# haoxiangsnr/Wave-U-Net-for-Speech-Enhancement

Hardware: AMD Instinct MI355X
Metric: 16384-sample frames/sec fwd+bwd, 12-level Wave-U-Net (higher is better)
Workload: dtype f32 (levels >= 16 samples: 3 x f16 MFMA on hi/lo fp16 halves, fp32 accumulate; the rest f32 MFMA); 1 GPU; unet_basic 12-level, 16384-sample frames, batch=64 per GPU, fp32, training-mode forward + smooth_l1 + backward + fused HIP Adam step (BASELINE.json configs[2]; configs[3] when n_gpus>1); global_batch=64, frame=16384, parallelism=dp1

## Files before the change

include/wunet_hip.h:

```cpp
#ifndef WUNET_HIP_H
#define WUNET_HIP_H

#include <stddef.h>

#ifdef __cplusplus
extern "C" {
#endif

typedef struct wunet_ctx wunet_ctx;

#define WUNET_OK 0
#define WUNET_E_ARG (-1)
#define WUNET_E_RUNTIME (-2)

#define WUNET_LOSS_MSE 0
#define WUNET_LOSS_L1 1
#define WUNET_LOSS_SMOOTH_L1 2

const char* wunet_last_error(void);

int wunet_create(int n_layers, int channels_interval, int batch, int length, wunet_ctx** out);
void wunet_destroy(wunet_ctx* ctx);

int wunet_set_h3(wunet_ctx* ctx, int enable);
// ... 13 lines not shown
                   float* const* grads, void* stream);
int wunet_backward_range(wunet_ctx* ctx, const float* noisy, const float* const* params,
                         const float* enhanced, const float* grad_enhanced, void* workspace,
                         float* const* grads, int layer_begin, int layer_end, void* stream);
int wunet_backward_range_async(wunet_ctx* ctx, const float* noisy, const float* const* params,
                               const float* enhanced, const float* grad_enhanced, void* workspace,
                               float* const* grads, int layer_begin, int layer_end, void* stream);
int wunet_backward_join(wunet_ctx* ctx, void* stream);
int wunet_backward_input(wunet_ctx* ctx, const float* noisy, const float* const* params, void* workspace,
                         float* grad_noisy, void* stream);

size_t wunet_loss_scratch_bytes(void);
int wunet_loss_forward(int kind, const float* clean, const float* enhanced, size_t n,
                       float* loss_out, void* scratch, void* stream);
int wunet_loss_backward(int kind, const float* clean, const float* enhanced, const float* grad_loss,
                        size_t n, float* grad_enhanced, void* stream);

int wunet_adam_step(int n_tensors, float* const* params, const float* const* grads, float* const* exp_avg,
                    float* const* exp_avg_sq, const size_t* numels, double lr, double beta1, double beta2, double eps,
                    long long step, double grad_scale, long long* step_dev, float* hyper_dev, void* stream);

int wunet_layer_info(const wunet_ctx* ctx, int layer, size_t* z_offset_floats, int* channels, int* length);
int wunet_num_conv_layers(const wunet_ctx* ctx);

int wunet_profile_enable(int on);
long long wunet_profile_collect(char* buf, size_t cap);
int wunet_debug_stamps(unsigned long long* out, int n);

#define WUNET_COMM_ID_BYTES 128
typedef struct wunet_comm wunet_comm;
int wunet_comm_unique_id(unsigned char* id );
int wunet_comm_create(const unsigned char* id, int world, int rank, wunet_comm** out);
int wunet_comm_allreduce_sum(wunet_comm* comm, float* buf, size_t count, void* stream);
int wunet_comm_world(const wunet_comm* comm);
void wunet_comm_destroy(wunet_comm* comm);

int wunet_crop_windows(const float* mixture_flat, const float* clean_flat, const long long* starts, long long total,
                       int batch, int length, float* mixture, float* clean, void* stream);

void wunet_debug_set_conv_trace(void* dev_buffer);

int wunet_op_conv1d(const float* x, const float* w, const float* bias, float* z,
                    int B, int Cin, int Cout, int L, int K, void* stream);
int wunet_op_conv1d_dgrad(const float* gz, const float* w, float* dx,
                          int B, int Cin, int Cout, int L, int K, void* stream);
int wunet_op_conv1d_wgrad(const float* gz, const float* x, float* dw,
// ... 14 lines not shown
```

wave-u-net-for-speech-enhancement_amd/_lib.py:

```python
import ctypes
import os

_HERE = os.path.dirname(os.path.abspath(__file__))
LIB_PATH = os.environ.get("WUNET_LIB_PATH") or os.path.join(_HERE, "csrc", "libwunet_hip.so")

EXPORTS = [
    "wunet_last_error", "wunet_create", "wunet_destroy", "wunet_workspace_bytes", "wunet_forward",
    "wunet_backward", "wunet_backward_range", "wunet_loss_scratch_bytes", "wunet_loss_forward",
    "wunet_loss_backward", "wunet_layer_info", "wunet_num_conv_layers", "wunet_op_conv1d",
    "wunet_op_conv1d_dgrad", "wunet_op_conv1d_wgrad", "wunet_profile_enable", "wunet_profile_collect",
    "wunet_adam_step", "wunet_set_h3", "wunet_op_conv1d_split", "wunet_op_conv1d_dgrad_split", "wunet_op_conv1d_wgrad_split",
    "wunet_backward_range_async", "wunet_backward_join", "wunet_debug_set_conv_trace", "wunet_crop_windows",
    "wunet_comm_unique_id", "wunet_comm_create", "wunet_comm_allreduce_sum", "wunet_comm_world", "wunet_comm_destroy",
    "wunet_debug_stamps", "wunet_set_bn_frozen", "wunet_backward_input",
]

_vp = ctypes.c_void_p
_i = ctypes.c_int
_sz = ctypes.c_size_t


def declare(lib):
    lib.wunet_last_error.restype = ctypes.c_char_p
    lib.wunet_last_error.argtypes = []
    lib.wunet_create.argtypes = [_i, _i, _i, _i, ctypes.POINTER(_vp)]
    lib.wunet_destroy.argtypes = [_vp]
    lib.wunet_destroy.restype = None
    lib.wunet_workspace_bytes.argtypes = [_vp, _i]
    lib.wunet_workspace_bytes.restype = _sz
    lib.wunet_forward.argtypes = [_vp, _vp, _vp, _vp, _vp, _i, _i, _vp, _vp, _vp]
    lib.wunet_backward.argtypes = [_vp, _vp, _vp, _vp, _vp, _vp, _vp, _vp]
    lib.wunet_backward_range.argtypes = [_vp, _vp, _vp, _vp, _vp, _vp, _vp, _i, _i, _vp]
    lib.wunet_backward_range_async.argtypes = [_vp, _vp, _vp, _vp, _vp, _vp, _vp, _i, _i, _vp]
    lib.wunet_backward_join.argtypes = [_vp, _vp]
    if hasattr(lib, "wunet_backward_input"):
        lib.wunet_backward_input.argtypes = [_vp, _vp, _vp, _vp, _vp, _vp]
    lib.wunet_loss_scratch_bytes.restype = _sz
    lib.wunet_loss_scratch_bytes.argtypes = []
    lib.wunet_loss_forward.argtypes = [_i, _vp, _vp, _sz, _vp, _vp, _vp]
    lib.wunet_loss_backward.argtypes = [_i, _vp, _vp, _vp, _sz, _vp, _vp]
    lib.wunet_layer_info.argtypes = [_vp, _i, ctypes.POINTER(_sz), ctypes.POINTER(_i), ctypes.POINTER(_i)]
    lib.wunet_num_conv_layers.argtypes = [_vp]
    for name in ("wunet_op_conv1d", "wunet_op_conv1d_split"):
        getattr(lib, name).argtypes = [_vp, _vp, _vp, _vp, _i, _i, _i, _i, _i, _vp]
    for name in ("wunet_op_conv1d_dgrad", "wunet_op_conv1d_wgrad", "wunet_op_conv1d_dgrad_split", "wunet_op_conv1d_wgrad_split"):
        getattr(lib, name).argtypes = [_vp, _vp, _vp, _i, _i, _i, _i, _i, _vp]
    lib.wunet_adam_step.argtypes = [_i, _vp, _vp, _vp, _vp, _vp, ctypes.c_double, ctypes.c_double, ctypes.c_double,
                                    ctypes.c_double, ctypes.c_longlong, ctypes.c_double, _vp, _vp, _vp]
    lib.wunet_set_h3.argtypes = [_vp, _i]
    if hasattr(lib, "wunet_set_bn_frozen"):
        lib.wunet_set_bn_frozen.argtypes = [_vp, _vp, _i]
    lib.wunet_profile_enable.argtypes = [_i]
    lib.wunet_profile_collect.argtypes = [ctypes.c_char_p, _sz]
    lib.wunet_profile_collect.restype = ctypes.c_longlong
    if hasattr(lib, "wunet_debug_stamps"):
        lib.wunet_debug_stamps.argtypes = [ctypes.POINTER(ctypes.c_ulonglong), _i]
        lib.wunet_debug_stamps.restype = _i
    lib.wunet_crop_windows.argtypes = [_vp, _vp, _vp, ctypes.c_longlong, _i, _i, _vp, _vp, _vp]
    lib.wunet_comm_unique_id.argtypes = [_vp]
    lib.wunet_comm_create.argtypes = [_vp, _i, _i, ctypes.POINTER(_vp)]
    lib.wunet_comm_allreduce_sum.argtypes = [_vp, _vp, _sz, _vp]
    lib.wunet_comm_world.argtypes = [_vp]
    lib.wunet_comm_destroy.argtypes = [_vp]
    lib.wunet_comm_destroy.restype = None
    lib.wunet_debug_set_conv_trace.argtypes = [_vp]
# ... 17 lines not shown
```

wave-u-net-for-speech-enhancement_amd/csrc/wunet_elementwise.h:

```cpp
#pragma once
#include "wunet_dev.h"

struct PackDesc {
    const float* w;
    float* dst;
    int Cout, Cin, taps;
    int M;
    int CP;
    int mtiles;
    int transposed;
};

#define WUNET_MAX_CONV_LAYERS 34
struct PackTable { PackDesc d[WUNET_MAX_CONV_LAYERS]; };

static __global__ __launch_bounds__(WUNET_THREADS) void pack_weights_kernel(PackTable tab)
{
    const PackDesc& d = tab.d[blockIdx.y];
    const int total = d.mtiles * d.CP * d.taps * 16;
    const int kc = d.transposed ? d.Cout : d.Cin;
    for (int idx = blockIdx.x * WUNET_THREADS + threadIdx.x; idx < total; idx += gridDim.x * WUNET_THREADS) {
        const int i = idx & 15;
        int r = idx >> 4;
        const int t = r % d.taps; r /= d.taps;
// ... 52 lines not shown
    const float* bias;
    const float* gamma;
    const float* beta;
    float* running_mean;
    float* running_var;
    long long* nbt;
    float* a;
    float* s;
    float* mean;
    float* rstd;
    int C;
    double count;
    int training;
};

struct BnFwdPre { float bias, gamma, beta, rmean, rvar; long long nbt; };
__device__ __forceinline__ BnFwdPre bn_finalize_preload(const BnFwdArgs& A, int c)
{
    BnFwdPre P;
    P.bias = A.bias[c]; P.gamma = A.gamma[c]; P.beta = A.beta[c]; P.rmean = A.running_mean[c]; P.rvar = A.running_var[c];
    P.nbt = c == 0 ? *A.nbt : 0;
    return P;
}
__device__ __forceinline__ void bn_finalize_core(const BnFwdArgs& A, int c, double s1, double s2, const BnFwdPre& P)
{
    const double m0 = s1 / A.count;
    double var = s2 / A.count - m0 * m0;
    var = var < 0.0 ? 0.0 : var;
    const double mean = m0 + (double)P.bias;
    const float rstd = (float)(1.0 / sqrt(var + 1e-5));
    const float a = P.gamma * rstd;
    const float sh = P.beta - (float)mean * a;
    A.a[c] = a;
    A.s[c] = sh;
    A.mean[c] = (float)mean;
    A.rstd[c] = rstd;
    const double unbiased = A.count > 1.0 ? var * A.count / (A.count - 1.0) : var;
    A.running_mean[c] = (float)(0.9 * (double)P.rmean + 0.1 * mean);
    A.running_var[c] = (float)(0.9 * (double)P.rvar + 0.1 * unbiased);
    if (c == 0) *A.nbt = P.nbt + 1;
}

__device__ __forceinline__ void bn_eval_core(const BnFwdArgs& A, int c)
{
    const float rstd = (float)(1.0 / sqrt((double)A.running_var[c] + 1e-5));
    const float a = A.gamma[c] * rstd;
    A.a[c] = a;
    A.s[c] = A.beta[c] - A.running_mean[c] * a;
}

struct BnEvalDesc { const float* gamma; const float* beta; const float* running_mean; const float* running_var; float* a; float* s; int C;
                    float* mean; float* rstd; };
struct BnEvalTable { BnEvalDesc d[WUNET_MAX_CONV_LAYERS]; };
static __global__ __launch_bounds__(WUNET_THREADS) void bn_eval_all_kernel(BnEvalTable T)
{
    const BnEvalDesc& d = T.d[blockIdx.y];
    const int c = blockIdx.x * WUNET_THREADS + threadIdx.x;
    if (c >= d.C) return;
    BnFwdArgs A{};
    A.gamma = d.gamma; A.beta = d.beta; A.running_mean = const_cast<float*>(d.running_mean); A.running_var = const_cast<float*>(d.running_var);
    A.a = d.a; A.s = d.s;
    bn_eval_core(A, c);
    if (d.mean) {
// ... 1040 lines not shown
```

wave-u-net-for-speech-enhancement_amd/csrc/wunet_forward.cpp:

```cpp
#include "wunet_host.h"
#include "wunet_elementwise.h"
#include "wunet_tiny.h"
#include "wunet_h3_elem.h"

using namespace wunet_host;

extern "C" {

int wunet_forward(wunet_ctx* c, const float* noisy, const float* const* params, float* const* running,
                  long long* const* nbt, int training, int save_for_backward, void* workspace, float* enhanced, void* stream)
{
    if (!c || !noisy || !params || !running || !nbt || !workspace || !enhanced) return fail(WUNET_E_ARG, "null argument");
    hipStream_t st = (hipStream_t)stream;
    float* ws = (float*)workspace;
    const bool packs_valid = !training && (save_for_backward & WUNET_FWD_PACKS_VALID) != 0;
    save_for_backward &= WUNET_FWD_SAVE;
    hipStream_t sd = st;
    float* const fslot = ws + c->fslot_off;
    auto frozen = [&](int i) { return training && c->any_frozen && i >= 0 && c->frozen[i] != 0; };
    auto skip_early = [&](const LayerPlan& dl) { return !frozen(dl.src0) && !frozen(dl.src1); };
    float* const enhanced_user = enhanced;
    if (c->padded) {
        if (hipMemsetAsync(ws + c->pad_in, 0, (size_t)c->B * c->T * sizeof(float), st) != hipSuccess ||
            hipMemcpy2DAsync(ws + c->pad_in, (size_t)c->T * sizeof(float), noisy, (size_t)c->Tt * sizeof(float), (size_t)c->Tt * sizeof(float),
                             (size_t)c->B, hipMemcpyDeviceToDevice, st) != hipSuccess)
            return fail(WUNET_E_RUNTIME, "padding the input failed");
        noisy = ws + c->pad_in;
        enhanced = ws + c->pad_out;
    }
    wunet_ctx::Side* fside = nullptr;
    if (training && c->NL > 1 && c->ly[0].first && !g_prof_on && !frozen(0)) {
        if (!side_stream_off()) fside = side_for_current_device(c);
        if (fside && (hipEventRecord(fside->ev_fork, st) != hipSuccess || hipStreamWaitEvent(fside->stream, fside->ev_fork, 0) != hipSuccess))
            return fail(WUNET_E_RUNTIME, "fork onto the side stream failed");
    }
    const hipStream_t pst = fside ? fside->stream : st;
    auto pack_fp32 = [&]() -> int {
        PackTable tab{};
        int nd = 0;
        for (int i = 0; i < c->NL; ++i) {
            const LayerPlan& l = c->ly[i];
            if (l.h3f || l.first) continue;
            PackDesc& d = tab.d[nd++];
// ... 111 lines not shown
            d.mean = ws + l.mean; d.rstd = ws + l.rstd;
            if (l.cout > maxc) maxc = l.cout;
        }
        if (nf > 0) {
            WUNET_LAUNCH(bn_eval_all_kernel, dim3((unsigned)((maxc + WUNET_THREADS - 1) / WUNET_THREADS), (unsigned)nf), dim3(WUNET_THREADS), 0, st, T);
            WUNET_CHECK_LAUNCH();
        }
    }
    for (int i = 0; i < c->NL; ++i) {
        const LayerPlan& l = c->ly[i];
        const bool fz = frozen(i);
        const bool bstats = training && !fz;
        if (!fpack_joined && i >= 1) {
            if (hipStreamWaitEvent(st, fside->ev_fpack, 0) != hipSuccess) return fail(WUNET_E_RUNTIME, "waiting for the weight packs failed");
            fpack_joined = true;
        }
        if (!fpack2_joined && i >= 1 && !l.h3f) {
            if (hipStreamWaitEvent(st, fside->ev_fpack2, 0) != hipSuccess) return fail(WUNET_E_RUNTIME, "waiting for the weight packs failed");
            fpack2_joined = true;
        }
        const float* xin = noisy;
        const bool use_u = i > 0 && (training ? l.h3u_train : l.h3u);
        const bool op_by_producer = !training && i > 0 && l.kind == LK_DECIM && c->ly[l.src0].evop;
        if (i > 0 && !use_u && !op_by_producer) {
            const LayerPlan& p = c->ly[l.src0];
            PrepArgs pa{};
            pa.z0 = ws + p.z; pa.a0 = ws + p.a; pa.s0 = ws + p.s; pa.x = ws + l.xin;
            pa.B = c->B; pa.C0 = l.c0; pa.C1 = l.cin - l.c0; pa.L = l.L; pa.logL = l.logL; pa.Lt = l.Lt;
            const size_t n4 = (size_t)c->B * l.cin * l.L / 4;
            size_t blocks = (n4 + WUNET_THREADS - 1) / WUNET_THREADS;
            if (blocks > 8192) blocks = 8192;
            if (l.h3x) {
                PrepH3Args ph{};
                ph.z0 = pa.z0; ph.a0 = pa.a0; ph.s0 = pa.s0;
                ph.xh = reinterpret_cast<wunet_half*>(ws + l.xh); ph.xl = reinterpret_cast<wunet_half*>(ws + l.xl);
                ph.B = c->B; ph.C0 = l.c0; ph.C1 = l.cin - l.c0; ph.C8 = (l.cin + 7) / 8; ph.L = l.L; ph.logL = l.logL; ph.Lt = l.Lt;
                ph.kind = l.kind == LK_UPCAT ? 1 : 0;
                ph.up_only = (l.kind == LK_UPCAT && l.skip_from > 0 && training && skip_early(l)) ? 1 : 0;
                ph.xb0 = fslot + (size_t)WUNET_SLOT_FLOATS * l.src0 + 4;
                ph.xb1 = l.kind == LK_UPCAT ? fslot + (size_t)WUNET_SLOT_FLOATS * l.src1 + 4 : nullptr;
                ph.xsc = fslot + (size_t)WUNET_SLOT_FLOATS * i;
                ph.bf = c->bf;
                if (l.kind == LK_DECIM && training) {
                    const int dj = 2 * c->n - i + 1;
                    if (dj < c->NL && c->ly[dj].skip_from == i && !c->ly[dj].h3u_train && skip_early(c->ly[dj])) {
                        const LayerPlan& dl = c->ly[dj];
                        ph.sh = reinterpret_cast<wunet_half*>(ws + dl.xh); ph.sl = reinterpret_cast<wunet_half*>(ws + dl.xl);
// ... 104 lines not shown
                                    split ? ws + c->spart_off : ws + l.z, (bstats && !split) ? ws + c->stats_off : nullptr, c->B, l.cout,
                                    l.cin, l.h3f_nch, l.L, st, ws + l.xzp, ev_epi ? ws + l.a : nullptr, ev_epi ? ws + l.s : nullptr, ev_epi ? xrows : nullptr, c->bf, l.h3f_ntt,
                                    evop ? &opo : nullptr);
            if (rc) return rc;
        } else if (tiny) {
            const size_t no = (size_t)c->B * l.cout * l.L;
            WUNET_LAUNCH(tiny_conv_kernel, dim3((unsigned)((no + WUNET_THREADS - 1) / WUNET_THREADS)), dim3(WUNET_THREADS), 0, st,
                         xin, params[4 * i], ws + c->spart_off, c->B, l.cin, l.cout, l.L, l.logL, l.taps, 0);
        } else {
            const ConvArgs a = make_conv_args(xin, l.cin, ws + c->wpkf_off + l.f_wpk, split ? nullptr : params[4 * i + 1],
                                              split ? ws + c->spart_off : ws + l.z, (bstats && !split) ? ws + c->stats_off : nullptr,
                                              c->B, l.cout, l.L, l.taps, l.f, (size_t)c->B * l.cout * l.L);
            int rc = launch_conv(l.taps, a, l.f, st);
            if (rc) return rc;
        }
        WUNET_CHECK_LAUNCH();
        if (ev_epi) {
        } else if (split) {
            const long long pos = (long long)c->B * l.L;
            int rs = (int)(pos / (bstats ? 2048 : 4096));
            if (rs < 1) rs = 1;
            if (rs > 64) rs = 64;
            b.rows = rs;
            WUNET_LAUNCH(conv_reduce_bn_kernel, dim3(l.cout, rs), dim3(WUNET_THREADS), 0, st, b, (const float*)(ws + c->spart_off),
                         tiny ? 1 : l.f.ksplit, (size_t)c->B * l.cout * l.L, ws + l.z, c->B, l.L, l.logL, ws + c->stats_off, l.Lt,
                         ev_need ? xrows : (float*)nullptr);
            if (rs > 1 && bstats) {
                WUNET_CHECK_LAUNCH();
                WUNET_LAUNCH(bn_finalize_fwd_kernel, dim3(l.cout), dim3(WUNET_THREADS), 0, st, b);
            }
        } else if (bstats) {
            WUNET_LAUNCH(bn_finalize_fwd_kernel, dim3(l.cout), dim3(WUNET_THREADS), 0, st, b);
        }
        WUNET_CHECK_LAUNCH();
        if (ev_need && !ev_epi && !split) {
            const size_t n4 = (size_t)c->B * l.cout * l.L / 4;
            size_t blocks = (n4 + WUNET_THREADS * 4 - 1) / (WUNET_THREADS * 4);
            if (blocks > 2048) blocks = 2048;
            if (blocks < 1) blocks = 1;
            WUNET_LAUNCH(act_max_kernel, dim3((unsigned)blocks), dim3(WUNET_THREADS), 0, st, (const float*)(ws + l.z), (const float*)(ws + l.a),
                         (const float*)(ws + l.s), l.cout, l.logL, n4, fslot + (size_t)WUNET_SLOT_FLOATS * i + 4);
            WUNET_CHECK_LAUNCH();
        }
    }
    if (!fpack_joined && hipStreamWaitEvent(st, fside->ev_fpack, 0) != hipSuccess) return fail(WUNET_E_RUNTIME, "waiting for the weight packs failed");
    if (!fpack2_joined && hipStreamWaitEvent(st, fside->ev_fpack2, 0) != hipSuccess) return fail(WUNET_E_RUNTIME, "waiting for the weight packs failed");
    {
        const LayerPlan& l = c->ly[c->NL - 1];
        HeadFwdArgs h{};
        h.z = ws + l.z; h.a = ws + l.a; h.s = ws + l.s; h.in = noisy;
        h.wh = params[4 * c->NL]; h.bh = params[4 * c->NL + 1]; h.out = enhanced;
        h.B = c->B; h.C = c->ci; h.T = c->T; h.logT = ilog2(c->T);
// ... 16 lines not shown
```

wave-u-net-for-speech-enhancement_amd/csrc/wunet_h3_elem.h:

```cpp
#pragma once
#include "wunet_elementwise.h"
#include "wunet_h3.h"

#define WUNET_SLOT_FLOATS 8
#define WUNET_WMAX_PARTS 64
struct ScaleDesc {
    const float* w; unsigned wn;
    const float* gamma; const float* beta; int C;
    float sqrtn;
    int frozen;
    float* zp0; float* zp1;
};
struct ScaleTable { ScaleDesc d[WUNET_MAX_CONV_LAYERS]; float* wmax; float* slots; int training; };

static __global__ __launch_bounds__(WUNET_THREADS) void h3_scales_kernel(ScaleTable T)
{
    __shared__ float red[WUNET_THREADS];
    const ScaleDesc& d = T.d[blockIdx.y];
    const int tid = threadIdx.x;
    if (d.w) {
        float m = 0.0f;
        for (unsigned i = blockIdx.x * WUNET_THREADS + tid; i < d.wn; i += gridDim.x * WUNET_THREADS) m = fmaxf(m, fabsf(d.w[i]));
        red[tid] = m;
        __syncthreads();
// ... 376 lines not shown
            if (src < total) {
                const size_t o = (4 * (base + wbase) + piece) * 8;
                wunet_sth8(hi + o, tb[0][wbase * 4 + piece]);
                if (!BFM) wunet_sth8(lo + o, tb[1][wbase * 4 + piece]);
            }
        }
        __syncthreads();
    }
}

struct PrepH3Args {
    const float* z0; const float* a0; const float* s0;
    const float* z1; const float* a1; const float* s1;
    wunet_half* xh; wunet_half* xl;
    int B, C0, C1, C8, L, logL, kind;
    float up_scale;
    wunet_half* sh; wunet_half* sl; int SC8, sc8off;
    int up_only;
    const float* xb0; const float* xb1; float* xsc;
    const float* ssb0; const float* ssb1;
    int bf;
    int Lt;
};

template <int MODE>
__global__ __launch_bounds__(WUNET_THREADS) void prep_h3_kernel(PrepH3Args A)
{
    constexpr int KIND = MODE >= 2 ? 1 : 0;
    constexpr bool SKIP_DST = MODE == 1, UP_ONLY = MODE == 3;
    const int Lh = A.L >> 1, C = A.C0 + A.C1;
    const int ngrp = UP_ONLY ? A.C0 / 8 : A.C8;
    const size_t total = (size_t)A.B * ngrp * A.L;
    float xs_ = 1.0f, xinv_ = 1.0f, ss_ = 1.0f;
    wunet_x_scale(A.xb0, A.xb1, xs_, xinv_);
    if (blockIdx.x == 0 && threadIdx.x == 0) { A.xsc[0] = xs_; A.xsc[1] = xinv_; }
    if (SKIP_DST) { float si_; wunet_x_scale(A.ssb0, A.ssb1, ss_, si_); }
    for (size_t i = (size_t)blockIdx.x * WUNET_THREADS + threadIdx.x; i < total; i += (size_t)gridDim.x * WUNET_THREADS) {
        const int p = (int)(i & (size_t)(A.L - 1));
        const unsigned grow = (unsigned)(i >> A.logL);
        const int b = (int)(grow / (unsigned)ngrp), c8 = (int)(grow - (unsigned)b * ngrp);
        const size_t row = (size_t)b * A.C8 + c8;
        int i0 = 0, i1 = 0;
        float l0 = 0.0f, l1 = 0.0f;
        if (KIND != 0) wunet_up_coord(p, A.Lt >> 1, A.up_scale, i0, i1, l0, l1);
        const int lane = (int)(threadIdx.x & 63);
        const int q0 = A.L >= 64 ? 2 * (p - lane) + lane : 2 * p;
// ... 18 lines not shown
                const float* zr = A.z0 + ((size_t)b * A.C0 + cc) * (size_t)(2 * A.L);
                za[e] = zr[2 * p];
                zb[e] = 0.0f;
                if (SKIP_DST) { zq[0][e] = zr[q0]; zq[1][e] = zr[q0 + qstep]; }
            } else {
                const bool up = UP_ONLY || cc < A.C0;
                from_up[e] = up;
                const int cu = up ? cc : 0, cs = up ? 0 : cc - A.C0;
                const float* zr = up ? A.z0 + ((size_t)b * A.C0 + cu) * Lh : A.z1 + ((size_t)b * A.C1 + cs) * A.L;
                za[e] = zr[up ? i0 : p];
                zb[e] = zr[up ? i1 : p];
                if (!vec_c) {
                    av[e] = up ? A.a0[cu] : A.a1[cs];
                    sv[e] = up ? A.s0[cu] : A.s1[cs];
                }
            }
        }
        {
            wunet_h8 h, l;
#pragma unroll
            for (int e = 0; e < 8; ++e) {
                const int c = c8 * 8 + e;
                float v;
                if (KIND == 0) v = wunet_lrelu(av[e] * za[e] + sv[e]);
                else {
                    const float u0 = wunet_lrelu(av[e] * za[e] + sv[e]), u1 = wunet_lrelu(av[e] * zb[e] + sv[e]);
                    v = from_up[e] ? l0 * u0 + l1 * u1 : u0;
                }
                if (c >= C || p >= A.Lt) v = 0.0f;
                wunet_half a, d;
                wunet_split_rt(A.bf, xs_ * v, a, d);
                wunet_put_half(h, e, a);
                wunet_put_half(l, e, d);
            }
            wunet_sth8(A.xh + (row * A.L + (size_t)p) * 8, h);
            if (!A.bf) wunet_sth8(A.xl + (row * A.L + (size_t)p) * 8, l);
        }
        if (SKIP_DST) {
            const size_t srow = (size_t)b * A.SC8 + A.sc8off + c8;
#pragma unroll
            for (int k = 0; k < 2; ++k) {
                const int q = q0 + k * qstep;
                wunet_h8 h, l;
#pragma unroll
                for (int e = 0; e < 8; ++e) {
                    const int c = c8 * 8 + e;
                    const float v = (c < C && q < 2 * A.Lt) ? wunet_lrelu(av[e] * zq[k][e] + sv[e]) : 0.0f;
                    wunet_half a, d;
                    wunet_split_rt(A.bf, ss_ * v, a, d);
                    wunet_put_half(h, e, a);
                    wunet_put_half(l, e, d);
                }
                wunet_sth8(A.sh + (srow * (size_t)(2 * A.L) + (size_t)q) * 8, h);
                if (!A.bf) wunet_sth8(A.sl + (srow * (size_t)(2 * A.L) + (size_t)q) * 8, l);
            }
        }
    }
}

struct PackH3Desc {
    const float* w;
    wunet_half* hi;
    wunet_half* lo;
    int Cout, Cin, taps;
    int rows, kch;
    int mtiles, nch;
    int transposed;
    const float* wmax;
    float* wsc;
    int bf;
    int ntt;
    int nfull, ns;
};
struct PackH3Table { PackH3Desc d[WUNET_MAX_CONV_LAYERS]; };

static __global__ __launch_bounds__(WUNET_THREADS) void pack_h3_kernel(PackH3Table tab)
{
    const PackH3Desc& d = tab.d[blockIdx.y];
// ... 36 lines not shown
```

wave-u-net-for-speech-enhancement_amd/csrc/wunet_host.h:

```cpp
#pragma once
#include <cstdarg>
#include <cmath>
#include <cstdio>
#include <cstdlib>
#include <cstring>
#include <map>
#include <mutex>
#include <string>
#include <vector>

#include "wunet_kernels.h"
#include "wunet_h3.h"
#include "wunet_h3u.h"
#include "wunet_launch.h"
#include "wunet_hip.h"

namespace wunet_host {

int fail(int code, const char* fmt, ...);
const char* last_error_text();

#define WUNET_CHECK_LAUNCH()                                                                   \
    do {                                                                                       \
        hipError_t e_ = hipGetLastError();                                                     \
// ... 35 lines not shown
    WgradCfg w;
    int f_rows;
    int a_split;
    size_t f_wpk, d_wpk;
    size_t z, a, s, mean, rstd, xin, g, dx, k1, k2, k3;
    size_t wl1;
    int evop;
    int h3f, h3d;
    int h3f_mrep, h3f_mtp, h3f_nch, h3d_mrep, h3d_mtp, h3d_nch;
    int h3f_ntt, h3d_ntt;
    int h3f_sps, h3d_sps;
    int first;
    int h3x;
    int skip_from;
    int h3w, h3w_mrep, h3w_mblocks, h3w_nblocks, h3w_ksplit, h3w_cps, h3w_tp;
    int h3w_xcd;
    int h3u, h3u_train;
    int feeds_h3;
    size_t xh, xl, xzp;
    size_t gzh, gzl, gzp;
    size_t h3f_wpk, h3d_wpk;
    int upt;
    size_t dxh, usp;
};

struct H3ConvPlan { int mrep, mtp, nch, sps, ksplit, ntiles, ntt; };
H3ConvPlan plan_h3_conv(int B, int L, int rows, int kch, int taps, const char* order_env, int bf = 0);
size_t h3d_smem(int nseg, int mrep, int bf, int mtp, int eval, int upt = 0);
int h3d_blocks_per_cu(int nseg, int mrep, int bf);
int h3_stage_count(int kch, int taps, int ntt);
void plan_h3_wgrad(LayerPlan& l, int B);
size_t h3w_part_stride(const LayerPlan& l);
bool up_pairs_regular(int Lin);
unsigned pack_gx();

}

struct wunet_ctx {
    int n, ci, B, T, NL;
    int Tt = 0;
    bool padded = false;
    size_t pad_in = 0, pad_out = 0, pad_gout = 0;
    std::vector<wunet_host::LayerPlan> ly;
    size_t stats_off, wpkf_off, spart_off, fwd_floats;
    size_t bmax_off, bound_off;
    size_t bpart_off, wgpart_off, wpkb_off, gh_off, hpart_off, hpart2_off, e0part_off, total_floats;
// ... 11 lines not shown
        const void* packed_ws = nullptr;
    };
    std::map<int, Side> side;
    std::mutex side_lock;
};

namespace wunet_host {

void layout_workspace(wunet_ctx* c);
int launch_split(const float* x, wunet_half* hi, wunet_half* lo, const float* sc, const float* xb0, const float* xb1, float* xsc,
                 int B, int C, int L, hipStream_t st, int bf = 0);
struct ConvH3OpOut { wunet_half* h; wunet_half* l; const float* wl1; const float* xmax; float* xsc; int C8; };
struct ConvH3Upt { int c0; float up_scale; float* uh_out; float* uh_spill; };
int launch_conv_h3(int taps, int mrep, int mtiles_p, int sps, const wunet_half* xh, const wunet_half* xl, const wunet_half* wh,
                   const wunet_half* wl, const float* bias, const float* sc, const float* sc2, float* out, float* stats, int B, int rows,
                   int kch, int nch, int L, hipStream_t st, const void* zpad, const float* ev_a = nullptr, const float* ev_s = nullptr,
                   float* xrows = nullptr, int bf = 0, int ntt = 0, const ConvH3OpOut* op = nullptr, const ConvH3Upt* upt = nullptr);
int launch_conv_h3u(const ConvH3uArgs& a, int mrep, int mtiles_p, int kch, hipStream_t st);
int launch_wgrad_h3(const LayerPlan& l, const wunet_half* xh, const wunet_half* xl, const wunet_half* gh, const wunet_half* gl,
                    const float* sc, const float* sc2, float* part, int B, hipStream_t st, int bf = 0);
int launch_backward_packs(wunet_ctx* c, const float* const* params, float* ws, hipStream_t st);
wunet_ctx::Side* side_for_current_device(wunet_ctx* c);
bool side_stream_off();

}
```

wave-u-net-for-speech-enhancement_amd/csrc/wunet_plan.cpp:

```cpp
#include "wunet_host.h"
#include "wunet_h3_elem.h"

namespace wunet_host {

namespace { thread_local std::string g_err; }

int fail(int code, const char* fmt, ...)
{
    char buf[512];
    va_list ap;
    va_start(ap, fmt);
    vsnprintf(buf, sizeof buf, fmt, ap);
    va_end(ap);
    g_err = buf;
    return code;
}

const char* last_error_text() { return g_err.c_str(); }

namespace {
struct ProfRec { std::string name; double flops; double bytes; hipEvent_t e0, e1; };
std::vector<ProfRec> g_prof;
}
bool g_prof_on = false;
// ... 259 lines not shown
    l.h3w_mblocks = round_up(mt, l.h3w_mrep) / l.h3w_mrep;
    l.h3w_nblocks = (l.cin + cib - 1) / cib;
    l.h3w_tp = 128;
    const bool sb2 = l.L >= 128 && ((l.taps == 5 && l.h3w_mrep <= 4) || (l.taps == 15 && l.h3w_mrep <= 3));
    const long long slots = 256LL * ((l.h3w_mrep <= 2 || sb2) ? 2 : 1);
    long long ks = slots / ((long long)l.h3w_mblocks * l.h3w_nblocks);
    if (ks < 1) ks = 1;
    const long long chunks = ((long long)B * l.L + l.h3w_tp - 1) / l.h3w_tp;
    if (ks > chunks) ks = chunks;
    {
        static const bool xcd_off = getenv("WUNET_WGRAD_XCD") != nullptr && atoi(getenv("WUNET_WGRAD_XCD")) == 0;
        const long long nyz = (long long)l.h3w_mblocks * l.h3w_nblocks, per_xcd = slots / 8;
        l.h3w_xcd = 0;
        if (!xcd_off && nyz > 1 && l.L >= 128) {
            if (((ks + 7) / 8) * nyz <= per_xcd) l.h3w_xcd = 1;
            else {
                const long long ks8 = (per_xcd / nyz) * 8;
                if (ks8 >= 8 && ks8 * 100 >= ks * 94) { ks = ks8; l.h3w_xcd = 1; }
            }
        }
    }
    l.h3w_cps = (int)((chunks + ks - 1) / ks);
    l.h3w_ksplit = (int)((chunks + l.h3w_cps - 1) / l.h3w_cps);
}

bool up_pairs_regular(int Lin)
{
    static std::mutex lock;
    static std::map<int, bool> seen;
    std::lock_guard<std::mutex> g(lock);
    auto it = seen.find(Lin);
    if (it != seen.end()) return it->second;
    bool ok = Lin >= 2;
    const int Lout = 2 * Lin;
    const float scale = (float)(Lin - 1) / (float)(Lout - 1);
    for (int j = 0; ok && j < Lout; ++j) {
        volatile float src = scale * (float)j;
        int a = (int)floorf(src);
        a = a > Lin - 1 ? Lin - 1 : a;
        float lam = src - (float)a;
        lam = lam < 0.0f ? 0.0f : (lam > 1.0f ? 1.0f : lam);
        if (j == 0) ok = a == 0 && lam == 0.0f;
        else ok = a == ((j - 1) >> 1) && (a < Lin - 1 || lam == 0.0f);
    }
    return seen[Lin] = ok;
}
// ... 83 lines not shown
            l.h3f_wpk = wfh; wfh += (size_t)l.h3f_mtp * l.h3f_nch * l.taps * 512;
        }
    }
    c->h3_wf_halfs = wfh;
    c->h3_wf_hi = off; off += align64((wfh + 1) / 2);
    c->h3_wf_lo = off; off += align64((wfh + 1) / 2);
    c->fslot_off = off; off += align64((size_t)WUNET_SLOT_FLOATS * c->NL);
    c->wmax_off = off; off += align64((size_t)WUNET_WMAX_PARTS * c->NL);
    for (int i = 0; i < c->NL; ++i) c->ly[i].evop = 0;
    for (int i = 1; i + 1 <= c->n; ++i) {
        LayerPlan& p = c->ly[i];
        const LayerPlan& q = c->ly[i + 1];
        if (p.h3f && !p.first && p.taps == 15 && p.L >= 256 && p.f.ksplit == 1 && p.h3f_mrep <= 4 && q.kind == LK_DECIM && q.src0 == i && q.h3f && q.h3x &&
            !c->bf && !c->padded && !getenv("WUNET_NO_EVOP"))
            p.evop = 1;
    }
    for (int i = 0; i < c->NL; ++i) c->ly[i].feeds_h3 = 0;
    for (int i = 1; i < c->NL; ++i) {
        const LayerPlan& l = c->ly[i];
        if (!l.h3f) continue;
        c->ly[l.src0].feeds_h3 = 1;
        if (l.kind == LK_UPCAT) c->ly[l.src1].feeds_h3 = 1;
    }
    if (c->padded) {
        c->pad_in = off; off += align64((size_t)B * T);
        c->pad_out = off; off += align64((size_t)B * T);
    }
    c->fwd_floats = off;

    size_t wpkb = 0, bpart_max = 0, wgpart_max = 0;
    for (int i = 0; i < c->NL; ++i) {
        LayerPlan& l = c->ly[i];
        l.g = off; off += align64((size_t)B * l.cout * l.L);
        l.dx = off; if (i > 0) off += align64((size_t)B * l.cin * l.L);
        l.k1 = off; off += align64(l.cout);
        l.k2 = off; off += align64(l.cout);
        l.k3 = off; off += align64(l.cout);
        l.d_wpk = wpkb;
        if (i > 0) wpkb += align64((size_t)l.d.mtiles_p * l.d.cp * l.taps * 16);
        if (l.h3w) plan_h3_wgrad(l, B);
        const size_t wg = l.h3w ? (size_t)l.h3w_ksplit * h3w_part_stride(l) : (size_t)l.w.rows * l.cout * l.cin * l.taps;
        if (wg > wgpart_max) wgpart_max = wg;
        long long sp = ((long long)B * l.L) / 4096;
        static const int a_cap_env = getenv("WUNET_A_CAP") ? atoi(getenv("WUNET_A_CAP")) : 128;
        const int a_cap = a_cap_env < 1 ? 1 : (a_cap_env > 256 ? 256 : a_cap_env);
        l.a_split = (int)(sp < 1 ? 1 : (sp > a_cap ? a_cap : sp));
// ... 111 lines not shown
        ctx->any_frozen = ctx->any_frozen || ctx->frozen[i];
    }
    return WUNET_OK;
}

void wunet_destroy(wunet_ctx* ctx)
{
    if (!ctx) return;
    for (auto& kv : ctx->side) {
        hipStreamDestroy(kv.second.stream); hipEventDestroy(kv.second.ev_fork); hipEventDestroy(kv.second.ev_join); hipEventDestroy(kv.second.ev_pack);
        hipEventDestroy(kv.second.ev_fpack); hipEventDestroy(kv.second.ev_fpack2);
    }
    delete ctx;
}

size_t wunet_workspace_bytes(const wunet_ctx* ctx, int with_backward)
{
    if (!ctx) return 0;
    return (with_backward ? ctx->total_floats : ctx->fwd_floats) * sizeof(float);
}

int wunet_num_conv_layers(const wunet_ctx* ctx) { return ctx ? ctx->NL : 0; }

int wunet_layer_info(const wunet_ctx* ctx, int layer, size_t* z_offset_floats, int* channels, int* length)
{
    if (!ctx || layer < 0 || layer >= ctx->NL) return fail(WUNET_E_ARG, "bad layer");
    if (z_offset_floats) *z_offset_floats = ctx->ly[layer].z;
    if (channels) *channels = ctx->ly[layer].cout;
    if (length) *length = ctx->ly[layer].L;
    return WUNET_OK;
}

}
```

Baseline: 12820 frames/s.

## Fuse split-K reduce, BN stats and next-layer operand prep for short layers

```diff
diff --git a/include/wunet_hip.h b/include/wunet_hip.h
--- a/include/wunet_hip.h
+++ b/include/wunet_hip.h
@@ -59,6 +59,9 @@
 
 int wunet_layer_info(const wunet_ctx* ctx, int layer, size_t* z_offset_floats, int* channels, int* length);
 int wunet_num_conv_layers(const wunet_ctx* ctx);
+int wunet_layer_operand_info(const wunet_ctx* ctx, int layer, size_t* a_offset_floats, size_t* s_offset_floats,
+                             size_t* operand_offset_floats, size_t* operand_lo_offset_floats, size_t* operand_floats,
+                             int* reduce_writes_operands);
 
 int wunet_profile_enable(int on);
 long long wunet_profile_collect(char* buf, size_t cap);
diff --git a/wave-u-net-for-speech-enhancement_amd/_lib.py b/wave-u-net-for-speech-enhancement_amd/_lib.py
--- a/wave-u-net-for-speech-enhancement_amd/_lib.py
+++ b/wave-u-net-for-speech-enhancement_amd/_lib.py
@@ -12,7 +12,7 @@
     "wunet_adam_step", "wunet_set_h3", "wunet_op_conv1d_split", "wunet_op_conv1d_dgrad_split", "wunet_op_conv1d_wgrad_split",
     "wunet_backward_range_async", "wunet_backward_join", "wunet_debug_set_conv_trace", "wunet_crop_windows",
     "wunet_comm_unique_id", "wunet_comm_create", "wunet_comm_allreduce_sum", "wunet_comm_world", "wunet_comm_destroy",
-    "wunet_debug_stamps", "wunet_set_bn_frozen", "wunet_backward_input",
+    "wunet_debug_stamps", "wunet_set_bn_frozen", "wunet_backward_input", "wunet_layer_operand_info",
 ]
 
 _vp = ctypes.c_void_p
@@ -41,6 +41,9 @@
     lib.wunet_loss_backward.argtypes = [_i, _vp, _vp, _vp, _sz, _vp, _vp]
     lib.wunet_layer_info.argtypes = [_vp, _i, ctypes.POINTER(_sz), ctypes.POINTER(_i), ctypes.POINTER(_i)]
     lib.wunet_num_conv_layers.argtypes = [_vp]
+    if hasattr(lib, "wunet_layer_operand_info"):
+        lib.wunet_layer_operand_info.argtypes = [_vp, _i, ctypes.POINTER(_sz), ctypes.POINTER(_sz), ctypes.POINTER(_sz), ctypes.POINTER(_sz),
+                                                 ctypes.POINTER(_sz), ctypes.POINTER(_i)]
     for name in ("wunet_op_conv1d", "wunet_op_conv1d_split"):
         getattr(lib, name).argtypes = [_vp, _vp, _vp, _vp, _i, _i, _i, _i, _i, _vp]
     for name in ("wunet_op_conv1d_dgrad", "wunet_op_conv1d_wgrad", "wunet_op_conv1d_dgrad_split", "wunet_op_conv1d_wgrad_split"):
diff --git a/wave-u-net-for-speech-enhancement_amd/csrc/wunet_elementwise.h b/wave-u-net-for-speech-enhancement_amd/csrc/wunet_elementwise.h
--- a/wave-u-net-for-speech-enhancement_amd/csrc/wunet_elementwise.h
+++ b/wave-u-net-for-speech-enhancement_amd/csrc/wunet_elementwise.h
@@ -98,7 +98,7 @@
     P.nbt = c == 0 ? *A.nbt : 0;
     return P;
 }
-__device__ __forceinline__ void bn_finalize_core(const BnFwdArgs& A, int c, double s1, double s2, const BnFwdPre& P)
+__device__ __forceinline__ void bn_finalize_core(const BnFwdArgs& A, int c, double s1, double s2, const BnFwdPre& P, float& a_out, float& s_out)
 {
     const double m0 = s1 / A.count;
     double var = s2 / A.count - m0 * m0;
@@ -115,6 +115,13 @@
     A.running_mean[c] = (float)(0.9 * (double)P.rmean + 0.1 * mean);
     A.running_var[c] = (float)(0.9 * (double)P.rvar + 0.1 * unbiased);
     if (c == 0) *A.nbt = P.nbt + 1;
+    a_out = a;
+    s_out = sh;
+}
+__device__ __forceinline__ void bn_finalize_core(const BnFwdArgs& A, int c, double s1, double s2, const BnFwdPre& P)
+{
+    float a, sh;
+    bn_finalize_core(A, c, s1, s2, P, a, sh);
 }
 
 __device__ __forceinline__ void bn_eval_core(const BnFwdArgs& A, int c)
diff --git a/wave-u-net-for-speech-enhancement_amd/csrc/wunet_forward.cpp b/wave-u-net-for-speech-enhancement_amd/csrc/wunet_forward.cpp
--- a/wave-u-net-for-speech-enhancement_amd/csrc/wunet_forward.cpp
+++ b/wave-u-net-for-speech-enhancement_amd/csrc/wunet_forward.cpp
@@ -19,6 +19,17 @@
     float* const fslot = ws + c->fslot_off;
     auto frozen = [&](int i) { return training && c->any_frozen && i >= 0 && c->frozen[i] != 0; };
     auto skip_early = [&](const LayerPlan& dl) { return !frozen(dl.src0) && !frozen(dl.src1); };
+    const bool tails = training && save_for_backward;
+    auto tail_on = [&](int p) { return tails && p >= 0 && c->ly[p].rtail && !frozen(p); };
+    auto served = [&](int x) {
+        const LayerPlan& l = c->ly[x];
+        if (x <= 0 || !tail_on(l.src0)) return false;
+        if (l.kind == LK_DECIM) return true;
+        if (l.kind != LK_UPCAT) return false;
+        if (l.h3x) return l.skip_from > 0 && skip_early(l);
+        return tail_on(l.src1) && skip_early(l);
+    };
+    auto fused = [&](int p) { return tail_on(p) && (p < c->n || served(p + 1)); };
     float* const enhanced_user = enhanced;
     if (c->padded) {
         if (hipMemsetAsync(ws + c->pad_in, 0, (size_t)c->B * c->T * sizeof(float), st) != hipSuccess ||
@@ -176,7 +187,9 @@
         const float* xin = noisy;
         const bool use_u = i > 0 && (training ? l.h3u_train : l.h3u);
         const bool op_by_producer = !training && i > 0 && l.kind == LK_DECIM && c->ly[l.src0].evop;
-        if (i > 0 && !use_u && !op_by_producer) {
+        const bool op_by_tail = served(i);
+        if (op_by_tail) xin = ws + l.xin;
+        if (i > 0 && !use_u && !op_by_producer && !op_by_tail) {
             const LayerPlan& p = c->ly[l.src0];
             PrepArgs pa{};
             pa.z0 = ws + p.z; pa.a0 = ws + p.a; pa.s0 = ws + p.s; pa.x = ws + l.xin;
@@ -327,12 +340,58 @@
             if (rs < 1) rs = 1;
             if (rs > 64) rs = 64;
             b.rows = rs;
-            WUNET_LAUNCH(conv_reduce_bn_kernel, dim3(l.cout, rs), dim3(WUNET_THREADS), 0, st, b, (const float*)(ws + c->spart_off),
-                         tiny ? 1 : l.f.ksplit, (size_t)c->B * l.cout * l.L, ws + l.z, c->B, l.L, l.logL, ws + c->stats_off, l.Lt,
-                         ev_need ? xrows : (float*)nullptr);
-            if (rs > 1 && bstats) {
-                WUNET_CHECK_LAUNCH();
-                WUNET_LAUNCH(bn_finalize_fwd_kernel, dim3(l.cout), dim3(WUNET_THREADS), 0, st, b);
+            if (fused(i)) {
+                ReduceOpsArgs o{};
+                o.bf = c->bf;
+                double obytes = 0.0;
+                const double hb = c->bf ? 2.0 : 4.0;
+                if (i < c->n) {
+                    const LayerPlan& q = c->ly[i + 1];
+                    if (q.h3x) {
+                        o.dh = reinterpret_cast<wunet_half*>(ws + q.xh); o.dl = reinterpret_cast<wunet_half*>(ws + q.xl);
+                        o.dC8 = (q.cin + 7) / 8; o.d_xb = fslot + (size_t)WUNET_SLOT_FLOATS * i + 4; o.d_xsc = fslot + (size_t)WUNET_SLOT_FLOATS * (i + 1);
+                    } else o.dx = ws + q.xin;
+                    obytes += (double)c->B * l.cout * q.L * (q.h3x ? hb : 4.0);
+                    const int dj = 2 * c->n - i;
+                    if (dj < c->NL && c->ly[dj].src1 == i) {
+                        const LayerPlan& dl = c->ly[dj];
+                        if (dl.h3x) {
+                            if (dl.skip_from == i + 1 && !dl.h3u_train && skip_early(dl)) {
+                                o.sh = reinterpret_cast<wunet_half*>(ws + dl.xh); o.sl = reinterpret_cast<wunet_half*>(ws + dl.xl);
+                                o.sC8 = (dl.cin + 7) / 8; o.sc8off = dl.c0 / 8;
+                                o.s_xb0 = fslot + (size_t)WUNET_SLOT_FLOATS * dl.src0 + 4; o.s_xb1 = fslot + (size_t)WUNET_SLOT_FLOATS * dl.src1 + 4;
+                                obytes += (double)c->B * l.cout * l.L * hb;
+                            }
+                        } else if (served(dj)) {
+                            o.sx = ws + dl.xin; o.sC = dl.cin; o.sc0 = dl.c0;
+                            obytes += (double)c->B * l.cout * l.L * 4.0;
+                        }
+                    }
+                } else {
+                    const LayerPlan& q = c->ly[i + 1];
+                    if (q.h3x) {
+                        o.uh = reinterpret_cast<wunet_half*>(ws + q.xh); o.ul = reinterpret_cast<wunet_half*>(ws + q.xl);
+                        o.uC8 = (q.cin + 7) / 8; o.u_xb0 = fslot + (size_t)WUNET_SLOT_FLOATS * q.src0 + 4;
+                        o.u_xb1 = fslot + (size_t)WUNET_SLOT_FLOATS * q.src1 + 4; o.u_xsc = fslot + (size_t)WUNET_SLOT_FLOATS * (i + 1);
+                    } else { o.ux = ws + q.xin; o.uC = q.cin; }
+                    o.up_scale = q.Lt > 1 ? (float)(q.Lt / 2 - 1) / (float)(q.Lt - 1) : 0.f;
+                    obytes += (double)c->B * l.cout * q.L * (q.h3x ? hb : 4.0);
+                }
+                const int ks = l.f.ksplit;
+                const size_t smem = ((size_t)WUNET_ROPS_HEAD_FLOATS + (size_t)c->B * l.L) * sizeof(float);
+                if (WUNET_ALLOW_BIG_LDS(conv_reduce_bn_ops_kernel, smem) != 0) return fail(WUNET_E_RUNTIME, "conv_reduce_bn_ops_kernel: %zu bytes of LDS refused", smem);
+                prof_begin(st, "conv_reduce_bn_ops_kernel", 0.0, 4.0 * c->B * l.cout * l.L * (ks + 1.0) + obytes);
+                WUNET_LAUNCH(conv_reduce_bn_ops_kernel, dim3(l.cout), dim3(WUNET_THREADS), smem, st, b, o, (const float*)(ws + c->spart_off), ks,
+                             (size_t)c->B * l.cout * l.L, ws + l.z, c->B, l.L, l.logL, l.Lt, rs);
+                prof_end(st);
+            } else {
+                WUNET_LAUNCH(conv_reduce_bn_kernel, dim3(l.cout, rs), dim3(WUNET_THREADS), 0, st, b, (const float*)(ws + c->spart_off),
+                             tiny ? 1 : l.f.ksplit, (size_t)c->B * l.cout * l.L, ws + l.z, c->B, l.L, l.logL, ws + c->stats_off, l.Lt,
+                             ev_need ? xrows : (float*)nullptr);
+                if (rs > 1 && bstats) {
+                    WUNET_CHECK_LAUNCH();
+                    WUNET_LAUNCH(bn_finalize_fwd_kernel, dim3(l.cout), dim3(WUNET_THREADS), 0, st, b);
+                }
             }
         } else if (bstats) {
             WUNET_LAUNCH(bn_finalize_fwd_kernel, dim3(l.cout), dim3(WUNET_THREADS), 0, st, b);
diff --git a/wave-u-net-for-speech-enhancement_amd/csrc/wunet_h3_elem.h b/wave-u-net-for-speech-enhancement_amd/csrc/wunet_h3_elem.h
--- a/wave-u-net-for-speech-enhancement_amd/csrc/wunet_h3_elem.h
+++ b/wave-u-net-for-speech-enhancement_amd/csrc/wunet_h3_elem.h
@@ -422,6 +422,24 @@
     int bf;
     int Lt;
 };
+
+#ifdef WUNET_EMU
+__device__ __forceinline__ float wunet_bn_act(float a, float z, float s) { return wunet_lrelu(a * z + s); }
+__device__ __forceinline__ float wunet_blend(float l0, float u0, float l1, float u1) { return l0 * u0 + l1 * u1; }
+__device__ __forceinline__ float wunet_blend32(float l0, float u0, float l1, float u1) { return l0 * u0 + l1 * u1; }
+#else
+__device__ __forceinline__ float wunet_bn_act(float a, float z, float s) { return wunet_lrelu(__builtin_fmaf(a, z, s)); }
+__device__ __forceinline__ float wunet_blend(float l0, float u0, float l1, float u1) { return __builtin_fmaf(l0, u0, l1 * u1); }
+__device__ __forceinline__ float wunet_blend32(float l0, float u0, float l1, float u1) { return __builtin_fmaf(l1, u1, l0 * u0); }
+#endif
+__device__ __forceinline__ float wunet_bn_act_up(float a, float s, float z0, float z1, float l0, float l1)
+{
+    return wunet_blend(l0, wunet_bn_act(a, z0, s), l1, wunet_bn_act(a, z1, s));
+}
+__device__ __forceinline__ float wunet_bn_act_up32(float a, float s, float z0, float z1, float l0, float l1)
+{
+    return wunet_blend32(l0, wunet_bn_act(a, z0, s), l1, wunet_bn_act(a, z1, s));
+}
 
 template <int MODE>
 __global__ __launch_bounds__(WUNET_THREADS) void prep_h3_kernel(PrepH3Args A)
@@ -486,10 +504,10 @@
             for (int e = 0; e < 8; ++e) {
                 const int c = c8 * 8 + e;
                 float v;
-                if (KIND == 0) v = wunet_lrelu(av[e] * za[e] + sv[e]);
+                if (KIND == 0) v = wunet_bn_act(av[e], za[e], sv[e]);
                 else {
-                    const float u0 = wunet_lrelu(av[e] * za[e] + sv[e]), u1 = wunet_lrelu(av[e] * zb[e] + sv[e]);
-                    v = from_up[e] ? l0 * u0 + l1 * u1 : u0;
+                    const float u0 = wunet_bn_act(av[e], za[e], sv[e]), u1 = wunet_bn_act(av[e], zb[e], sv[e]);
+                    v = from_up[e] ? wunet_blend(l0, u0, l1, u1) : u0;
                 }
                 if (c >= C || p >= A.Lt) v = 0.0f;
                 wunet_half a, d;
@@ -509,7 +527,7 @@
 #pragma unroll
                 for (int e = 0; e < 8; ++e) {
                     const int c = c8 * 8 + e;
-                    const float v = (c < C && q < 2 * A.Lt) ? wunet_lrelu(av[e] * zq[k][e] + sv[e]) : 0.0f;
+                    const float v = (c < C && q < 2 * A.Lt) ? wunet_bn_act(av[e], zq[k][e], sv[e]) : 0.0f;
                     wunet_half a, d;
                     wunet_split_rt(A.bf, ss_ * v, a, d);
                     wunet_put_half(h, e, a);
@@ -518,6 +536,216 @@
                 wunet_sth8(A.sh + (srow * (size_t)(2 * A.L) + (size_t)q) * 8, h);
                 if (!A.bf) wunet_sth8(A.sl + (srow * (size_t)(2 * A.L) + (size_t)q) * 8, l);
             }
+        }
+    }
+}
+
+struct ReduceOpsArgs {
+    wunet_half* dh; wunet_half* dl; float* dx; int dC8;
+    const float* d_xb; float* d_xsc;
+    wunet_half* sh; wunet_half* sl; float* sx; int sC8, sc8off, sC, sc0;
+    const float* s_xb0; const float* s_xb1;
+    wunet_half* uh; wunet_half* ul; float* ux; int uC8, uC; float up_scale;
+    const float* u_xb0; const float* u_xb1; float* u_xsc;
+    int bf;
+};
+#define WUNET_ROPS_HEAD_FLOATS 1060
+#define WUNET_ROPS_MAX_CHUNKS 64
+
+static __global__ __launch_bounds__(WUNET_THREADS) void conv_reduce_bn_ops_kernel(BnFwdArgs A, ReduceOpsArgs O, const float* __restrict__ part,
+                                                                            int ksplit, size_t split_stride, float* __restrict__ z, int B,
+                                                                            int L, int logL, int Lt, int nchunk)
+{
+    WUNET_DYN_SMEM(smem);
+    double* const red = reinterpret_cast<double*>(smem);
+    double* const wsum = red + 16;
+    float* const as = reinterpret_cast<float*>(wsum + WUNET_ROPS_MAX_CHUNKS * 8);
+    float* const zs = smem + WUNET_ROPS_HEAD_FLOATS;
+    const int c = blockIdx.x, tid = threadIdx.x;
+    const float bias = A.bias[c];
+    const BnFwdPre P = bn_finalize_preload(A, c);
+    const int total4 = (B * L) >> 2;
+    int p4 = tid;
+    for (; p4 + 3 * WUNET_THREADS < total4; p4 += 4 * WUNET_THREADS) {
+        size_t off[4];
+        wunet_f4 v[4];
+#pragma unroll
+        for (int i = 0; i < 4; ++i) {
+            const int p = (p4 + i * WUNET_THREADS) << 2;
+            off[i] = ((size_t)(p >> logL) * A.C + c) * L + (p & (L - 1));
+            v[i] = wunet_f4{0.f, 0.f, 0.f, 0.f};
+        }
+        int k = 0;
+        for (; k + 4 <= ksplit; k += 4) {
+            wunet_f4 t[4][4];
+#pragma unroll
+            for (int i = 0; i < 4; ++i)
+#pragma unroll
+                for (int q = 0; q < 4; ++q) t[i][q] = wunet_ld4(part + off[i] + (size_t)(k + q) * split_stride);
+#pragma unroll
+            for (int i = 0; i < 4; ++i)
+#pragma unroll
+                for (int j = 0; j < 4; ++j) { v[i][j] += t[i][0][j]; v[i][j] += t[i][1][j]; v[i][j] += t[i][2][j]; v[i][j] += t[i][3][j]; }
+        }
+        for (; k < ksplit; ++k) {
+            wunet_f4 t[4];
+#pragma unroll
+            for (int i = 0; i < 4; ++i) t[i] = wunet_ld4(part + off[i] + (size_t)k * split_stride);
+#pragma unroll
+            for (int i = 0; i < 4; ++i)
+#pragma unroll
+                for (int j = 0; j < 4; ++j) v[i][j] += t[i][j];
+        }
+#pragma unroll
+        for (int i = 0; i < 4; ++i) {
+            wunet_f4 o;
+#pragma unroll
+            for (int j = 0; j < 4; ++j) o[j] = v[i][j] + bias;
+            wunet_st4(z + off[i], o);
+            wunet_st4(zs + ((p4 + i * WUNET_THREADS) << 2), v[i]);
+        }
+    }
+    for (; p4 < total4; p4 += WUNET_THREADS) {
+        const int p = p4 << 2;
+        const size_t off = ((size_t)(p >> logL) * A.C + c) * L + (p & (L - 1));
+        const wunet_f4 v = wunet_sum_splits4(part + off, ksplit, split_stride);
+        wunet_f4 o;
+#pragma unroll
+        for (int j = 0; j < 4; ++j) o[j] = v[j] + bias;
+        wunet_st4(z + off, o);
+        wunet_st4(zs + p, v);
+    }
+    __syncthreads();
+    const int per = (total4 + nchunk - 1) / nchunk;
+    double r1 = 0.0, r2 = 0.0;
+    if (nchunk == 1) {
+        for (int q4 = tid; q4 < total4; q4 += WUNET_THREADS) {
+            const wunet_f4 v = wunet_ld4(zs + (q4 << 2));
+            const int l = (q4 << 2) & (L - 1);
+#pragma unroll
+            for (int j = 0; j < 4; ++j)
+                if (l + j < Lt) {
+                    r1 += (double)v[j];
+                    r2 += (double)v[j] * (double)v[j];
+                }
+        }
+    } else {
+        for (int y = 0; y < nchunk; ++y) {
+            const int beg = y * per, end = beg + per < total4 ? beg + per : total4;
+            double s1 = 0.0, s2 = 0.0;
+            for (int q4 = beg + tid; q4 < end; q4 += WUNET_THREADS) {
+                const wunet_f4 v = wunet_ld4(zs + (q4 << 2));
+                const int l = (q4 << 2) & (L - 1);
+#pragma unroll
+                for (int j = 0; j < 4; ++j)
+                    if (l + j < Lt) {
+                        s1 += (double)v[j];
+                        s2 += (double)v[j] * (double)v[j];
+                    }
+            }
+#pragma unroll
+            for (int m = 32; m > 0; m >>= 1) {
+                s1 += wunet_shfl_xor_d(s1, m);
+                s2 += wunet_shfl_xor_d(s2, m);
+            }
+            if ((tid & 63) == 0) {
+                wsum[y * 8 + (tid >> 6)] = s1;
+                wsum[y * 8 + 4 + (tid >> 6)] = s2;
+            }
+        }
+        __syncthreads();
+        if (tid < nchunk) {
+            const double* w = wsum + tid * 8;
+            const double c1 = (w[0] + w[1]) + (w[2] + w[3]), c2 = (w[4] + w[5]) + (w[6] + w[7]);
+            r1 += (double)(float)c1;
+            r2 += (double)(float)c2;
+        }
+    }
+    block_sum2(r1, r2, red);
+    if (tid == 0) {
+        float a_, s_;
+        bn_finalize_core(A, c, r1, r2, P, a_, s_);
+        as[0] = a_;
+        as[1] = s_;
+    }
+    __syncthreads();
+    const float a = as[0], s = as[1];
+    const int e = c & 7, g = c >> 3;
+    if (O.dh) {
+        const int Ld = L >> 1, Ltd = Lt >> 1, nd = B * Ld;
+        float xs, xinv;
+        wunet_x_scale(O.d_xb, nullptr, xs, xinv);
+        if (c == 0 && tid == 0) { O.d_xsc[0] = xs; O.d_xsc[1] = xinv; }
+        for (int i = tid; i < nd; i += WUNET_THREADS) {
+            const int b = i >> (logL - 1), l = i & (Ld - 1);
+            float v = wunet_bn_act(a, zs[(b << logL) + 2 * l] + bias, s);
+            if (l >= Ltd) v = 0.0f;
+            wunet_half hi, lo;
+            wunet_split_rt(O.bf, xs * v, hi, lo);
+            const size_t o = (((size_t)b * O.dC8 + g) * Ld + l) * 8 + e;
+            O.dh[o] = hi;
+            if (!O.bf) O.dl[o] = lo;
+        }
+    } else if (O.dx) {
+        const int Ld = L >> 1, Ltd = Lt >> 1, nd = B * Ld;
+        for (int i = tid; i < nd; i += WUNET_THREADS) {
+            const int b = i >> (logL - 1), l = i & (Ld - 1);
+            float v = wunet_bn_act(a, zs[(b << logL) + 2 * l] + bias, s);
+            if (l >= Ltd) v = 0.0f;
+            O.dx[((size_t)b * A.C + c) * Ld + l] = v;
+        }
+    }
+    if (O.sh) {
+        float ss, si;
+        wunet_x_scale(O.s_xb0, O.s_xb1, ss, si);
+        const int n = B * L;
+        for (int i = tid; i < n; i += WUNET_THREADS) {
+            const int b = i >> logL, q = i & (L - 1);
+            const float v = q < Lt ? wunet_bn_act(a, zs[i] + bias, s) : 0.0f;
+            wunet_half hi, lo;
+            wunet_split_rt(O.bf, ss * v, hi, lo);
+            const size_t o = (((size_t)b * O.sC8 + O.sc8off + g) * L + q) * 8 + e;
+            O.sh[o] = hi;
+            if (!O.bf) O.sl[o] = lo;
+        }
+    } else if (O.sx) {
+        const int n = B * L;
+        for (int i = tid; i < n; i += WUNET_THREADS) {
+            const int b = i >> logL, q = i & (L - 1);
+            const float v = q < Lt ? wunet_bn_act(a, zs[i] + bias, s) : 0.0f;
+            O.sx[((size_t)b * O.sC + O.sc0 + c) * L + q] = v;
+        }
+    }
+    if (O.uh) {
+        float xs, xinv;
+        wunet_x_scale(O.u_xb0, O.u_xb1, xs, xinv);
+        if (c == 0 && tid == 0) { O.u_xsc[0] = xs; O.u_xsc[1] = xinv; }
+        const int n = B * 2 * L;
+        for (int i = tid; i < n; i += WUNET_THREADS) {
+            const int b = i >> (logL + 1), p = i & (2 * L - 1);
+            int i0, i1;
+            float l0, l1;
+            wunet_up_coord(p, Lt, O.up_scale, i0, i1, l0, l1);
+            const float* zr = zs + (b << logL);
+            float v = wunet_bn_act_up(a, s, zr[i0] + bias, zr[i1] + bias, l0, l1);
+            if (p >= 2 * Lt) v = 0.0f;
+            wunet_half hi, lo;
+            wunet_split_rt(O.bf, xs * v, hi, lo);
+            const size_t o = (((size_t)b * O.uC8 + g) * (size_t)(2 * L) + p) * 8 + e;
+            O.uh[o] = hi;
+            if (!O.bf) O.ul[o] = lo;
+        }
+    } else if (O.ux) {
+        const int n = B * 2 * L;
+        for (int i = tid; i < n; i += WUNET_THREADS) {
+            const int b = i >> (logL + 1), p = i & (2 * L - 1);
+            int i0, i1;
+            float l0, l1;
+            wunet_up_coord(p, Lt, O.up_scale, i0, i1, l0, l1);
+            const float* zr = zs + (b << logL);
+            float v = wunet_bn_act_up32(a, s, zr[i0] + bias, zr[i1] + bias, l0, l1);
+            if (p >= 2 * Lt) v = 0.0f;
+            O.ux[((size_t)b * O.uC + c) * (size_t)(2 * L) + p] = v;
         }
     }
 }
diff --git a/wave-u-net-for-speech-enhancement_amd/csrc/wunet_host.h b/wave-u-net-for-speech-enhancement_amd/csrc/wunet_host.h
--- a/wave-u-net-for-speech-enhancement_amd/csrc/wunet_host.h
+++ b/wave-u-net-for-speech-enhancement_amd/csrc/wunet_host.h
@@ -81,6 +81,7 @@
     size_t h3f_wpk, h3d_wpk;
     int upt;
     size_t dxh, usp;
+    int rtail;
 };
 
 struct H3ConvPlan { int mrep, mtp, nch, sps, ksplit, ntiles, ntt; };
@@ -138,5 +139,6 @@
 int launch_backward_packs(wunet_ctx* c, const float* const* params, float* ws, hipStream_t st);
 wunet_ctx::Side* side_for_current_device(wunet_ctx* c);
 bool side_stream_off();
+int reduce_ops_max_len();
 
 }
diff --git a/wave-u-net-for-speech-enhancement_amd/csrc/wunet_plan.cpp b/wave-u-net-for-speech-enhancement_amd/csrc/wunet_plan.cpp
--- a/wave-u-net-for-speech-enhancement_amd/csrc/wunet_plan.cpp
+++ b/wave-u-net-for-speech-enhancement_amd/csrc/wunet_plan.cpp
@@ -305,6 +305,12 @@
     }
     l.h3w_cps = (int)((chunks + ks - 1) / ks);
     l.h3w_ksplit = (int)((chunks + l.h3w_cps - 1) / l.h3w_cps);
+}
+
+int reduce_ops_max_len()
+{
+    static const int v = getenv("WUNET_REDUCE_OPS") ? atoi(getenv("WUNET_REDUCE_OPS")) : 256;
+    return v < 0 ? 0 : v;
 }
 
 bool up_pairs_regular(int Lin)
@@ -434,6 +440,20 @@
         c->ly[l.src0].feeds_h3 = 1;
         if (l.kind == LK_UPCAT) c->ly[l.src1].feeds_h3 = 1;
     }
+    for (int i = 0; i < c->NL; ++i) c->ly[i].rtail = 0;
+    {
+        const int max_len = reduce_ops_max_len();
+        for (int i = 1; i + 1 < c->NL && max_len > 0; ++i) {
+            LayerPlan& p = c->ly[i];
+            const LayerPlan& q = c->ly[i + 1];
+            const bool through_reduce = !p.first && p.L >= 4 && (p.f.ksplit > 1 || c->padded);
+            if (!through_reduce || p.L > max_len || (size_t)B * p.L * sizeof(float) > 64 * 1024) continue;
+            if (q.src0 != i || q.L < 4 || q.h3u_train) continue;
+            if (q.h3x && ((p.cout & 7) || (q.kind == LK_UPCAT && (q.c0 & 7)))) continue;
+            if (q.kind == LK_UPCAT && !(q.h3x ? q.skip_from > 0 : c->ly[q.src1].rtail != 0)) continue;
+            p.rtail = 1;
+        }
+    }
     if (c->padded) {
         c->pad_in = off; off += align64((size_t)B * T);
         c->pad_out = off; off += align64((size_t)B * T);
@@ -591,6 +611,22 @@
 
 int wunet_num_conv_layers(const wunet_ctx* ctx) { return ctx ? ctx->NL : 0; }
 
+int wunet_layer_operand_info(const wunet_ctx* ctx, int layer, size_t* a_offset_floats, size_t* s_offset_floats,
+                             size_t* operand_offset_floats, size_t* operand_lo_offset_floats, size_t* operand_floats,
+                             int* reduce_writes_operands)
+{
+    if (!ctx || layer < 0 || layer >= ctx->NL) return fail(WUNET_E_ARG, "bad layer");
+    const LayerPlan& l = ctx->ly[layer];
+    if (a_offset_floats) *a_offset_floats = l.a;
+    if (s_offset_floats) *s_offset_floats = l.s;
+    const bool none = layer == 0 || (!l.h3f && l.h3x);
+    if (operand_offset_floats) *operand_offset_floats = l.h3f ? l.xh : l.xin;
+    if (operand_lo_offset_floats) *operand_lo_offset_floats = l.h3f ? l.xl : 0;
+    if (operand_floats) *operand_floats = none ? 0 : l.h3f ? (size_t)ctx->B * ((l.cin + 7) / 8) * l.L * 4 : (size_t)ctx->B * l.cin * l.L;
+    if (reduce_writes_operands) *reduce_writes_operands = l.rtail;
+    return WUNET_OK;
+}
+
 int wunet_layer_info(const wunet_ctx* ctx, int layer, size_t* z_offset_floats, int* channels, int* length)
 {
     if (!ctx || layer < 0 || layer >= ctx->NL) return fail(WUNET_E_ARG, "bad layer");
```

Result: slower. 12650 frames/s (-1.3%).
